# Vchitect/Latte

Measured on AMD Instinct MI355X. Metric: denoising steps/sec, higher is better.
Workload: dtype f16; 1 GPU; Latte-XL/2 FaceForensics (uncond) 16x256x256 -> latents 16x4x32x32, DDIM on the '250' respacing, random-init weights; per_gpu_batch=8, global_batch=8, parallelism=dp1 (independent samples)

## Files before the change

latte_amd/csrc/engine.cpp:

```cpp
#include <algorithm>
#include <cmath>
#include <cstdio>
#include <cstring>
#include <string>
#include <vector>

#include "event_profile.h"
#include "plan.h"
#include "weight_store.h"

namespace latte {

static thread_local std::string g_last_error;
static std::atomic<int> g_debug_choice[DBG_NUM_CHOICES];
int debug_choice(DebugChoice c) { return g_debug_choice[c].load(std::memory_order_relaxed); }
int set_debug_choice(const char* name, int value) {
  static const char* const names[DBG_NUM_CHOICES] = {"attn_variant", "xattn_flash", "tn_kernel", "tn_wn", "attn_bwd_tiles", "conv_kernel", "vae_split", "gated_rmw_shape"};
  static const int allowed[DBG_NUM_CHOICES][4] = {{1, 5, 12, 13}, {1, 0, 0, 0}, {4, 0, 0, 0}, {4, 0, 0, 0}, {1, 2, 0, 0}, {1, 2, 3, 4}, {0, 0, 0, 0}, {1, 2, 0, 0}};
  for (int i = 0; i < DBG_NUM_CHOICES; ++i) {
    if (name && std::string(name) == names[i]) {
      bool ok = value == 0;
      for (int k = 0; k < 4; ++k) ok = ok || (allowed[i][k] != 0 && value == allowed[i][k]);
      ok = ok || (i == DBG_VAE_SPLIT && (value >> 24) == 1);
      if (!ok) return -1;
// ... 199 lines not shown
  } else {
    if ((rc = launch_patch_embed(x, e->pe_wt, e->pe_b, e->pos, e->xres, B * F, e->Cin, e->H, c.patch_size, D, st))) return rc;
  }
  tm.mark(C_PATCH);
  int gsplit = cfg_dup ? e->guided_split : 0;
  if (dt != LATTE_DTYPE_F16) gsplit &= 3;
  if ((gsplit & 16) && !gemm_lo4_ok(M, e->Hm, D)) gsplit = (gsplit & ~16) | 8;
  if (gsplit & 16) gsplit &= ~10;
  if (gsplit & 4) gsplit &= ~1;
  if (gsplit & 8) gsplit &= ~2;
  if ((gsplit & 4) && !gemm_lo8_ok(M, D, D)) gsplit = (gsplit & ~4) | 1;
  if ((gsplit & 8) && !gemm_lo8_ok(M, e->Hm, D)) gsplit = (gsplit & ~8) | 2;
  if ((gsplit & 3) && (uint64_t)e->rows_pad * 2 * D * 2 >= (1ull << 32)) gsplit &= ~3;
  if (gsplit) gsplit = ensure_split_weights(e, gsplit, st);
  int gactive = gsplit & 26;

  for (int i = 0; i < c.depth; ++i) {
    const bool spatial = (i % 2) == 0;
    const BlockW& w = e->blocks[i];
    const float* mb = modp + (size_t)i * 6 * D;
    bool split_proj = false;
    const int fc2_variant = e->gemm_variant_of[3] ? e->gemm_variant_of[3] : e->gemm_variant;
    const bool te_in_fc2 = e->fc2_temp_embed && c.depth > 1 && gated_gemm_takes_te(e, M, D, e->Hm, fc2_variant);
    const float* te = (i == 1 && !te_in_fc2) ? e->temp : nullptr;
    if ((rc = launch_ln_modulate(e->xres, e->xres, e->xn, mb, mb + D, mstride, M, D, rps, te, T, F, dt, st))) return rc;
    tm.mark(C_LN);
    GemmArgs g{};
    g.M = M; g.rows_per_sample = rps; g.gate_stride = mstride; g.rmw_mode = e->gated_rmw_shape;
    const half_t* attn_out = e->xn;
    if (((e->fuse_qkv_attn >> (spatial ? 0 : 1)) & 1) && qkv_attention_fusable(D, c.num_heads, e->hd, F, T, spatial ? 0 : 1, M)) {
      QkvAttnArgs qa{};
      qa.xn = e->xn; qa.w = w.qkv_w; qa.bias = w.qkv_b; qa.out = e->qkv; qa.B = B; qa.F = F; qa.T = T; qa.D = D;
      qa.heads = c.num_heads; qa.hd = e->hd; qa.mode = spatial ? 0 : 1; qa.scale = 1.0f / std::sqrt((float)e->hd);
      qa.flags = ((e->fuse_qkv_attn >> 2) & 7) ^ 7;
      split_proj = gsplit & 5;
      qa.out_split = (gsplit & 4) ? 2 : (gsplit & 1);
      qa.out8 = e->lo8;
      gactive |= gsplit & 5;
      if ((rc = launch_qkv_attention(qa, dt, st))) return rc;
      tm.mark(spatial ? C_QKVATTN_S : C_QKVATTN_T);
      attn_out = e->qkv;
    } else {
      g.A = e->xn; g.W = w.qkv_w; g.bias = w.qkv_b; g.out = e->qkv; g.N = 3 * D; g.K = D;
      if ((rc = launch_gemm(g, EPI_BIAS_H16, dt, e->gemm_variant_of[0] ? e->gemm_variant_of[0] : e->gemm_variant, st))) return rc;
      tm.mark(C_QKV);
      AttnArgs a{};
      a.qkv = e->qkv; a.out = e->xn; a.heads = c.num_heads; a.hd = e->hd; a.D = D;
      a.sample_stride = rps; a.scale = 1.0f / std::sqrt((float)e->hd);
      if (spatial) { a.num_seq = B * F; a.L = T; a.U = F; a.seq_stride = T; a.row_stride = 1; }
      else         { a.num_seq = B * T; a.L = F; a.U = T; a.seq_stride = 1; a.row_stride = T; }
      if (gsplit & 4) {
        a.out8 = e->lo8;
        split_proj = true;
        gactive |= 4;
      }
      if ((rc = launch_attention(a, dt, st))) return rc;
      tm.mark(spatial ? C_ATTN_S : C_ATTN_T);
    }
    g.A = attn_out; g.W = w.proj_w; g.bias = w.proj_b; g.out = e->xres; g.gate = mb + 2 * D; g.N = D; g.K = D; g.tag = 0;
    if (split_proj && (gsplit & 4)) { g.A8 = e->lo8; g.W8 = w.proj_w8; }
    else if (split_proj) { g.W = w.proj_w2; g.K = 2 * D; }
    if ((rc = gated_gemm(e, g, dt, e->gemm_variant_of[1] ? e->gemm_variant_of[1] : e->gemm_variant, st))) return rc;
    g.A8 = nullptr; g.W8 = nullptr;
    tm.mark(C_PROJ);
    const int split_fc1 = (gsplit & 16) ? 3 : (gsplit & 8) ? 2 : (gsplit & 2) ? 1 : 0;
    if (split_fc1 == 3) rc = launch_ln_modulate_split4(e->xres, e->xn, e->lo4, e->lo4s, mb + 3 * D, mb + 4 * D, mstride, M, D, rps, dt, st);
    else rc = launch_ln_modulate(e->xres, e->xres, split_fc1 == 1 ? e->xn2 : e->xn, mb + 3 * D, mb + 4 * D, mstride, M, D, rps, nullptr, T, F, dt, st,
// ... 368 lines not shown
  const std::string k = name;
  if (k == "gemm_variant") {
    if (value < 0 || (value > 13 && value != 18 && value != 19)) return fail(LATTE_ERR_INVALID, "gemm_variant must be 0..13, 18 or 19");
    const int bn = value >= 7 && value <= 9 ? gemm_tile_n((int)value) / 4 : gemm_tile_n((int)value);
    if (value != 0 && ((3 * e->D) % bn || e->D % bn || e->Hm % bn))
      return fail(LATTE_ERR_INVALID, "gemm_variant: every N of the model must be a multiple of the tile width");
    e->gemm_variant = (int)value;
    return LATTE_OK;
  }
  for (int gi = 0; gi < 4; ++gi) {
    static const char* names[4] = {"gemm_variant_qkv", "gemm_variant_proj", "gemm_variant_fc1", "gemm_variant_fc2"};
    if (k == names[gi]) {
      if (value < 0 || (value > 13 && value != 18 && value != 19)) return fail(LATTE_ERR_INVALID, "gemm_variant_*: must be 0..13, 18 or 19");
      e->gemm_variant_of[gi] = (int)value;
      return LATTE_OK;
    }
  }
  if (k == "gated_split_k") {
    if (value < 0 || value > 4) return fail(LATTE_ERR_INVALID, "gated_split_k: 0 (rule), 1 (off) or 2..4 splits");
    e->gated_split_k = (int)value;
    return LATTE_OK;
  }
  if (k == "gated_rmw_shape") {
    if (value < 0 || value > 1) return fail(LATTE_ERR_INVALID, "gated_rmw_shape: 0 (fragment-wise) or 1 (line-wise residual accesses of the gated GEMMs)");
    e->gated_rmw_shape = (int)value;
    return LATTE_OK;
  }
  if (k == "fc2_temp_embed") {
    if (value < 0 || value > 1) return fail(LATTE_ERR_INVALID, "fc2_temp_embed: 0 (LayerNorm pass adds temp_embed) or 1 (the first block's fc2 epilogue does)");
    e->fc2_temp_embed = (int)value;
    return LATTE_OK;
  }
  if (k == "fuse_qkv_attn") {
    if (value < 0 || value > 31)
      return fail(LATTE_ERR_INVALID, "fuse_qkv_attn: bit 0 = spatial blocks, bit 1 = temporal blocks, bits 2-4 = schedule features off (0..31)");
    e->fuse_qkv_attn = (int)value;
    return LATTE_OK;
  }
  if (k == "guided_split") {
    if (value < 0 || value > 31)
      return fail(LATTE_ERR_INVALID, "guided_split: bit 0 / 1 = attention output / fc1 operand as f16 split pairs, bit 2 / 3 = the same with an fp8 remainder, bit 4 = fc1's operand with an fp4 remainder, in guided calls (0..31)");
    e->guided_split = (int)value;
    return LATTE_OK;
  }
  if (k == "seed") {
    e->seed = (uint64_t)value;
    e->rng_offset = 0;
    return LATTE_OK;
  }
  if (k == "train_timesteps") {
    if (value < 1 || value > (1 << 30)) return fail(LATTE_ERR_INVALID, "train_timesteps: the number of trained timesteps, >= 1");
    e->train_timesteps = (int)value;
    return LATTE_OK;
  }
  return fail(LATTE_ERR_INVALID, "set_option: unknown option '" + k + "'");
}

int latte_engine_get_option(const latte_engine_t* e, const char* name, int64_t* value) {
  if (!e || !name || !value) return fail(LATTE_ERR_INVALID, "get_option: null argument");
  const std::string k = name;
  if (k == "gemm_variant") *value = e->gemm_variant;
  else if (k == "gemm_variant_qkv") *value = e->gemm_variant_of[0];
  else if (k == "gemm_variant_proj") *value = e->gemm_variant_of[1];
  else if (k == "gemm_variant_fc1") *value = e->gemm_variant_of[2];
  else if (k == "gemm_variant_fc2") *value = e->gemm_variant_of[3];
  else if (k == "gated_split_k") *value = e->gated_split_k;
  else if (k == "gated_rmw_shape") *value = e->gated_rmw_shape;
  else if (k == "fc2_temp_embed") *value = e->fc2_temp_embed;
// ... 408 lines not shown
```

latte_amd/csrc/qkv_attn.hip:

```cpp
#include <type_traits>

#include "common.h"
#include "mfma_util.h"

namespace latte {
namespace {

constexpr int RPQ = 144, RPV = 160;
[[maybe_unused]] constexpr int Q_OFF = 0;
constexpr int K_OFF = 256 * RPQ, V_OFF = 2 * 256 * RPQ, IMG_END = V_OFF + 256 * RPV;
constexpr int A0_OFF = 0, A1_OFF = 61440, B1_OFF = 94208, B0_OFF = 122880, BIAS_OFF = B0_OFF + 224 * 128;
constexpr int FUSED_LDS = BIAS_OFF + 288 * 4;

__device__ __forceinline__ void rows_transpose4(unsigned int& x0, unsigned int& x1, unsigned int& x2, unsigned int& x3) {
  typedef __attribute__((ext_vector_type(2))) unsigned int u2;
  const u2 a = __builtin_amdgcn_permlane32_swap(x0, x2, false, false);
  const u2 b = __builtin_amdgcn_permlane32_swap(x1, x3, false, false);
  const u2 c = __builtin_amdgcn_permlane16_swap(a[0], b[0], false, false);
  const u2 d = __builtin_amdgcn_permlane16_swap(a[1], b[1], false, false);
  x0 = c[0]; x1 = c[1]; x2 = d[0]; x3 = d[1];
}

template <int HD, int DT, int MODE, int FLAGS, int SPLIT = 0>
__global__ void __launch_bounds__(512) qkv_attn_kernel(QkvAttnArgs a) {
  constexpr bool EARLY = (FLAGS & 1) != 0, PRIO = (FLAGS & 2) != 0;
  constexpr int NQ = 3 * HD;
  constexpr int NPAD = (NQ + 31) / 32 * 32;
  constexpr int FN = NPAD / 32;
  constexpr int B_MAIN = NPAD / 8 / 4;
  constexpr int GPM = HD / 8;
  constexpr int KS = (HD + 31) / 32, DF = (HD + 15) / 16, NCH = HD / 8;
  static_assert(NPAD <= 224 && NQ <= 288 && HD % 8 == 0 && A1_OFF >= 256 * 128 && B1_OFF - A1_OFF == 256 * 128 && B1_OFF + NPAD * 128 <= B0_OFF && IMG_END <= B0_OFF && K_OFF >= 256 * 128,
                "LDS plan");

  extern __shared__ __attribute__((aligned(16))) char smem[];
  const int lane = threadIdx.x & 63;
  const int wave = __builtin_amdgcn_readfirstlane(threadIdx.x >> 6);
  const int grp = wave >> 2, w4 = wave & 3, wm = w4 >> 1, wn = w4 & 1;
  const int D = a.D, T = a.T, F = a.F;
  const int out_ld = SPLIT == 1 ? 2 * D : D;
  const unsigned row_bytes = (unsigned)D * 2u;
  const int nk = D / 64;

  const int S = MODE == 0 ? a.B * F : a.B * (T >> 4);
  const bool xmap = (S & 7) == 0;
  const bool hmap = (a.flags & 4) != 0 && a.heads == 16 && xmap;
  const int xcd = blockIdx.x & 7;
  int it = xmap ? (int)(blockIdx.x >> 3) : (int)blockIdx.x;
  const int it_step = xmap ? (int)(gridDim.x >> 3) : (int)gridDim.x;
  const int it_end = xmap ? (S >> 3) * a.heads : S * a.heads;

  const __amdgpu_buffer_rsrc_t rsA =
      __builtin_amdgcn_make_buffer_rsrc((void*)a.xn, 0, (unsigned)((size_t)a.B * F * T) * row_bytes, 0x00020000);
  const __amdgpu_buffer_rsrc_t rsB = __builtin_amdgcn_make_buffer_rsrc((void*)a.w, 0, (unsigned)(3 * D) * row_bytes, 0x00020000);

  const int lrow = lane >> 3, cpos = lane & 7;
  const unsigned swz16 = (unsigned)((cpos ^ ((((w4 & 1) << 2) + (lrow >> 1)) & 7)) << 4);
  const unsigned voff_b = (unsigned)lrow * row_bytes + swz16;
// ... 97 lines not shown
    asm volatile("s_waitcnt lgkmcnt(0)" ::: "memory");
    __builtin_amdgcn_s_barrier();
    dma_a_half(cur, 1, 1);
    if (grp == 0) dma_b_all(cur, 1, 1);
    if (grp == 1) __builtin_amdgcn_s_barrier();
    for (int kt = 0; kt < nk; ++kt) {
      const char* sbuf_a = smem + ((kt & 1) ? A1_OFF : A0_OFF);
      const char* sbuf_b = smem + ((kt & 1) ? B1_OFF : B0_OFF);
      u32x4 bf[2][FN], af[2][4];
#pragma unroll
      for (int ks = 0; ks < 2; ++ks) {
#pragma unroll
        for (int j = 0; j < FN; ++j) bf[ks][j] = *(const u32x4*)(sbuf_b + ((b_off + j * 2048) ^ (ks << 6)));
#pragma unroll
        for (int i = 0; i < 4; ++i) af[ks][i] = *(const u32x4*)(sbuf_a + ((a_off + i * 2048) ^ (ks << 6)));
      }
      asm volatile("s_waitcnt lgkmcnt(0)" ::: "memory");
      __builtin_amdgcn_s_barrier();
      __builtin_amdgcn_s_setprio(1);
#pragma unroll
      for (int ks = 0; ks < 2; ++ks)
#pragma unroll
        for (int i = 0; i < 4; ++i)
#pragma unroll
          for (int j = 0; j < FN; ++j) acc[i][j] = mfma16<DT>(bf[ks][j], af[ks][i], acc[i][j]);
      __builtin_amdgcn_s_setprio(0);
      asm volatile("s_waitcnt vmcnt(0)" ::: "memory");
      __builtin_amdgcn_s_barrier();
      if (kt + 2 < nk) {
        dma_a_half(cur, kt + 2, kt & 1);
        if (grp == 0) dma_b_all(cur, kt + 2, kt & 1);
      }
    }
    if (grp == 0) __builtin_amdgcn_s_barrier();
    LATTE_PHASE(0)

    {
#pragma unroll
      for (int j = 0; j < FN; ++j) {
        const int n0 = wn * (NPAD / 2) + j * 16 + g * 4;
        if (n0 < NQ) {
          const int mat = n0 >= 2 * HD ? 2 : (n0 >= HD ? 1 : 0);
          const int d = n0 - mat * HD;
          const float4 b4 = *(const float4*)(smem + BIAS_OFF + n0 * 4);
          char* dst = smem + (mat == 2 ? V_OFF + (grp * 128 + wm * 64 + fr) * RPV : mat * K_OFF + (grp * 128 + wm * 64 + fr) * RPQ) + d * 2;
#pragma unroll
          for (int i = 0; i < 4; ++i) {
            const u32x2 pk = {pack2<DT>(acc[i][j][0] + b4.x, acc[i][j][1] + b4.y), pack2<DT>(acc[i][j][2] + b4.z, acc[i][j][3] + b4.w)};
            *(u32x2*)(dst + i * 16 * (mat == 2 ? RPV : RPQ)) = pk;
          }
        }
      }
    }
    __syncthreads();
    LATTE_PHASE(1)

    if (a.dbg_qkv != nullptr) {
      for (int idx = threadIdx.x; idx < 256 * 3 * NCH; idx += 512) {
        const int r = idx / (3 * NCH), rem = idx - r * (3 * NCH), mat = rem / NCH, ch = rem - mat * NCH;
        const int grow = MODE == 0 ? row_base + r : row_base + (r & 15) * T + (r >> 4);
        *(u32x4*)(a.dbg_qkv + (size_t)grow * (3 * D) + mat * D + head * HD + ch * 8) = *(const u32x4*)(smem + (mat == 2 ? V_OFF + r * RPV : mat * K_OFF + r * RPQ) + ch * 16);
      }
    }

    const char* q_img = smem;
    const char* k_img = smem + K_OFF;
    const char* v_img = smem + V_OFF;
    const float c = a.scale * 1.4426950408889634f;
    if constexpr (PRIO) {
      if (grp == 0) __builtin_amdgcn_s_setprio(2);
    }
    if constexpr (MODE == 0) {
      constexpr int NKT = 16;
      const int q0 = wave * 32;
      const char* kbase = k_img + fr * RPQ + g * 16;
      const char* vbase = v_img + (4 * g + (fr >> 2)) * RPV + (fr & 3) * 8;
      constexpr int NG = 2;
      {
        u32x4 qf[NG][KS];
#pragma unroll
        for (int gq = 0; gq < NG; ++gq)
#pragma unroll
          for (int ks = 0; ks < KS; ++ks) {
            const int ch = g + 4 * ks;
// ... 55 lines not shown
        for (int gq = 0; gq < NG; ++gq)
#pragma unroll
          for (int d = 0; d < DF; ++d) o[gq][d] = (f32x4){0.f, 0.f, 0.f, 0.f};
        u32x4 vfr[2][DF];
        auto load_v = [&](int ks2, u32x4 (&dst)[DF]) {
#pragma unroll
          for (int d = 0; d < DF; ++d) {
            const u32x2 lo = lds_tr16(vbase + (32 * ks2) * RPV + d * 32);
            const u32x2 hi = lds_tr16(vbase + (32 * ks2 + 16) * RPV + d * 32);
            dst[d] = (u32x4){lo[0], lo[1], hi[0], hi[1]};
          }
        };
        load_v(0, vfr[0]);
#pragma unroll
        for (int ks2 = 0; ks2 < NKT / 2; ++ks2) {
          if (ks2 + 1 < NKT / 2) load_v(ks2 + 1, vfr[(ks2 + 1) & 1]);
          u32x4 pb[NG];
#pragma unroll
          for (int gq = 0; gq < NG; ++gq)
            pb[gq] = (u32x4){pack2<DT>(st[gq][2 * ks2][0], st[gq][2 * ks2][1]), pack2<DT>(st[gq][2 * ks2][2], st[gq][2 * ks2][3]),
                             pack2<DT>(st[gq][2 * ks2 + 1][0], st[gq][2 * ks2 + 1][1]),
                             pack2<DT>(st[gq][2 * ks2 + 1][2], st[gq][2 * ks2 + 1][3])};
          __builtin_amdgcn_sched_barrier(0);
#pragma unroll
          for (int d = 0; d < DF; ++d)
#pragma unroll
            for (int gq = 0; gq < NG; ++gq) o[gq][d] = mfma16<DT>(vfr[ks2 & 1][d], pb[gq], o[gq][d]);
          __builtin_amdgcn_sched_barrier(0);
        }
#pragma unroll
        for (int gq = 0; gq < NG; ++gq) {
          half_t* orow = a.out + (size_t)(row_base + q0 + gq * 16 + fr) * out_ld + head * HD;
          unsigned int l8w[DF];
#pragma unroll
          for (int d = 0; d < DF; ++d) {
            const int dd = 16 * d + 4 * g;
            l8w[d] = 0u;
            if (dd < HD) {
              if constexpr (SPLIT == 1) {
                unsigned int h0_, l0_, h1_, l1_;
                split2<DT>(o[gq][d][0] * inv[gq], o[gq][d][1] * inv[gq], h0_, l0_);
                split2<DT>(o[gq][d][2] * inv[gq], o[gq][d][3] * inv[gq], h1_, l1_);
                const u32x2 hi = {h0_, h1_}, lo = {l0_, l1_};
                *(u32x2*)(orow + dd) = hi;
                *(u32x2*)(orow + D + dd) = lo;
              } else if constexpr (SPLIT == 2) {
                unsigned int h0_, h1_;
                l8w[d] = split8_f16(o[gq][d][0] * inv[gq], o[gq][d][1] * inv[gq], o[gq][d][2] * inv[gq], o[gq][d][3] * inv[gq], h0_, h1_);
                *(u32x2*)(orow + dd) = (u32x2){h0_, h1_};
              } else {
                const u32x2 pk = {pack2<DT>(o[gq][d][0] * inv[gq], o[gq][d][1] * inv[gq]),
                                  pack2<DT>(o[gq][d][2] * inv[gq], o[gq][d][3] * inv[gq])};
                *(u32x2*)(orow + dd) = pk;
              }
            }
          }
          if constexpr (SPLIT == 2) {
            unsigned char* o8 = a.out8 + (size_t)(row_base + q0 + gq * 16 + fr) * D + head * HD;
            rows_transpose4(l8w[0], l8w[1], l8w[2], l8w[3]);
            *(u32x4*)(o8 + 16 * g) = (u32x4){l8w[0], l8w[1], l8w[2], l8w[3]};
            if constexpr (DF > 4) { if (64 + 4 * g < HD) *(unsigned int*)(o8 + 64 + 4 * g) = l8w[4]; }
          }
        }
      }
    } else {
      f32x4 st2[2];
#pragma unroll
      for (int s2 = 0; s2 < 2; ++s2) {
        const int p = wave * 2 + s2;
        u32x4 qf[KS], kf[KS];
#pragma unroll
        for (int ks = 0; ks < KS; ++ks) {
          const int ch = g + 4 * ks;
          qf[ks] = *(const u32x4*)(q_img + (16 * p + fr) * RPQ + ch * 16);
          kf[ks] = *(const u32x4*)(k_img + (16 * p + fr) * RPQ + ch * 16);
          if (ch >= NCH) {
            qf[ks] = (u32x4){0u, 0u, 0u, 0u};
            kf[ks] = (u32x4){0u, 0u, 0u, 0u};
          }
        }
        st2[s2] = (f32x4){0.f, 0.f, 0.f, 0.f};
#pragma unroll
        for (int ks = 0; ks < KS; ++ks) st2[s2] = mfma16<DT>(kf[ks], qf[ks], st2[s2]);
      }
      early_fill();
#pragma unroll
      for (int s2 = 0; s2 < 2; ++s2) {
        const int p = wave * 2 + s2;
        f32x4 st = st2[s2];
        float mx = NEG_BIG;
#pragma unroll
        for (int r = 0; r < 4; ++r) mx = fmaxf(mx, st[r]);
        mx = fmaxf(mx, __shfl_xor(mx, 16, 64));
        mx = fmaxf(mx, __shfl_xor(mx, 32, 64));
        const float nm = -mx * c;
// ... 39 lines not shown
              *(u32x2*)(orow + dd) = pk;
            }
          }
        }
        if constexpr (SPLIT == 2) {
          unsigned char* o8 = a.out8 + (size_t)(row_base + fr * T + p) * D + head * HD;
          rows_transpose4(l8w[0], l8w[1], l8w[2], l8w[3]);
          *(u32x4*)(o8 + 16 * g) = (u32x4){l8w[0], l8w[1], l8w[2], l8w[3]};
          if constexpr (DF > 4) { if (64 + 4 * g < HD) *(unsigned int*)(o8 + 64 + 4 * g) = l8w[4]; }
        }
      }
    }
    if constexpr (PRIO) __builtin_amdgcn_s_setprio(0);
    asm volatile("s_waitcnt lgkmcnt(0)" ::: "memory");
    __builtin_amdgcn_s_barrier();
    LATTE_PHASE(2)
    tacc[3] += 1;
    if (!has_next) break;
    if (!filled_next) {
      fill_first(nxt);
      side = fetch_side(nxt);
    }
    cur = nxt;
    it = it_next;
  }
#undef LATTE_PHASE
  if (trace && lane == 0) {
    long long* o = a.dbg_trace + wave * 4;
#pragma unroll
    for (int i = 0; i < 4; ++i) o[i] = tacc[i];
  }
}

template <int HD, int DT, int MODE, int FLAGS, int SPLIT = 0>
int launch_one(const QkvAttnArgs& a, dim3 grid, hipStream_t st) {
  return launch_lds<qkv_attn_kernel<HD, DT, MODE, FLAGS, SPLIT>>(grid, dim3(512), FUSED_LDS, st, a);
}

template <int HD, int DT>
int launch_mode(const QkvAttnArgs& a, hipStream_t st) {
  const int S = a.mode == 0 ? a.B * a.F : a.B * (a.T >> 4);
  const int units = S * a.heads;
  const dim3 grid(units >= 256 ? 256 : (units + 7) / 8 * 8);
  if (a.out_split == 2) {
    if constexpr (DT == LATTE_DTYPE_F16) {
      if (!a.out8) return fail(LATTE_ERR_INVALID, "fused qkv + attention: out_split 2 needs out8");
      return a.mode == 0 ? launch_one<HD, DT, 0, 3, 2>(a, grid, st) : launch_one<HD, DT, 1, 1, 2>(a, grid, st);
    } else {
      return fail(LATTE_ERR_INVALID, "fused qkv + attention: the fp8-remainder output is f16 only");
    }
  }
  if (a.out_split)
    return a.mode == 0 ? launch_one<HD, DT, 0, 3, 1>(a, grid, st) : launch_one<HD, DT, 1, 1, 1>(a, grid, st);
  if (a.mode == 0) {
    switch (a.flags & 3) {
      case 0: return launch_one<HD, DT, 0, 0>(a, grid, st);
      case 1: return launch_one<HD, DT, 0, 1>(a, grid, st);
      case 2: return launch_one<HD, DT, 0, 2>(a, grid, st);
      default: return launch_one<HD, DT, 0, 3>(a, grid, st);
    }
  }
  return (a.flags & 1) ? launch_one<HD, DT, 1, 1>(a, grid, st) : launch_one<HD, DT, 1, 0>(a, grid, st);
}

}

bool qkv_attention_fusable(int D, int heads, int hd, int F, int T, int mode, int64_t rows) {
  if (heads * hd != D || (hd != 64 && hd != 72) || D % 64 != 0 || D < 128) return false;
  if ((uint64_t)rows * D * 2 >= (1ull << 32) || (uint64_t)3 * D * D * 2 >= (1ull << 32)) return false;
  if (mode == 0) return T == 256;
  return F == 16 && T % 16 == 0;
}

int launch_qkv_attention(const QkvAttnArgs& a, int dtype, hipStream_t st) {
  if (!qkv_attention_fusable(a.D, a.heads, a.hd, a.F, a.T, a.mode, (int64_t)a.B * a.F * a.T))
    return fail(LATTE_ERR_INVALID, "fused qkv + attention: shape not supported (need T == 256 spatial / F == 16 temporal, hd 64 | 72)");
  if (dtype == LATTE_DTYPE_BF16) return a.hd == 64 ? launch_mode<64, LATTE_DTYPE_BF16>(a, st) : launch_mode<72, LATTE_DTYPE_BF16>(a, st);
  if (dtype == LATTE_DTYPE_F16) return a.hd == 64 ? launch_mode<64, LATTE_DTYPE_F16>(a, st) : launch_mode<72, LATTE_DTYPE_F16>(a, st);
  return fail(LATTE_ERR_INVALID, "fused qkv + attention: unknown dtype");
}

}
```

latte_amd/csrc/t2v_engine.cpp:

```cpp
#include <algorithm>
#include <cmath>
#include <cstring>
#include <string>
#include <vector>

#include "../../include/latte_amd.h"
#include "plan.h"
#include "weight_store.h"

using namespace latte;

namespace {

enum T2VKind { TK_F32, TK_F32_TRANSPOSE, TK_H16 };

struct T2VBlock {
  half_t *qkv_w, *o_w, *q2_w, *kv2_w, *o2_w, *fc1_w, *fc2_w;
  float *qkv_b, *o_b, *q2_b, *kv2_b, *o2_b, *fc1_b, *fc2_b;
};

void sincos_1d(int dim, const std::vector<double>& pos, std::vector<double>& out ) {
  const int half = dim / 2, n = (int)pos.size();
  out.assign((size_t)n * dim, 0.0);
  for (int m = 0; m < n; ++m)
// ... 201 lines not shown
  LATTE_HIP(hipDeviceSynchronize());
  *out = e;
  return LATTE_OK;
}

void latte_t2v_destroy(latte_t2v_t* e) {
  delete e;
}

int latte_t2v_num_keys(const latte_t2v_t* e) { return e ? e->weights.size() : 0; }
const char* latte_t2v_key(const latte_t2v_t* e, int i) { return e ? e->weights.key(i) : nullptr; }

int latte_t2v_load_tensor(latte_t2v_t* e, const char* key, const float* data, int64_t numel, int on_device, void* stream) {
  if (!e || !key || !data) return fail(LATTE_ERR_INVALID, "t2v_load_tensor: null argument");
  hipStream_t st = (hipStream_t)stream;
  WeightSlot* slot = nullptr;
  const float* src = nullptr;
  int rc = e->weights.begin_load("t2v_load_tensor", key, data, numel, on_device, st, &slot, &src);
  if (rc || slot->optional) return rc;
  WeightSlot& s = *slot;
  switch (s.kind) {
    case TK_F32: LATTE_HIP(hipMemcpyAsync(s.dst, src, sizeof(float) * numel, hipMemcpyDeviceToDevice, st)); break;
    case TK_F32_TRANSPOSE: rc = launch_transpose_f32(src, (float*)s.dst, s.rows, s.cols, st); break;
    case TK_H16: rc = launch_convert_f32_to_h16(src, (half_t*)s.dst, numel, e->cfg.compute_dtype, st); break;
  }
  if (rc || (rc = e->weights.end_load(s, on_device, st))) return rc;
  e->txt_batch = 0;
  return LATTE_OK;
}

int latte_t2v_set_option(latte_t2v_t* e, const char* name, int64_t value) {
  if (!e || !name) return fail(LATTE_ERR_INVALID, "t2v_set_option: null argument");
  if (std::string(name) == "fuse_qkv_attn") {
    if (value < 0 || value > 31) return fail(LATTE_ERR_INVALID, "fuse_qkv_attn: bit 0 = spatial blocks, bit 1 = temporal blocks, bits 2-3 = schedule variant");
    e->fuse_qkv_attn = (int)value;
    return LATTE_OK;
  }
  return fail(LATTE_ERR_INVALID, std::string("t2v_set_option: unknown option '") + name + "'");
}

int latte_t2v_check_weights(latte_t2v_t* e) {
  if (!e) return fail(LATTE_ERR_INVALID, "t2v_check_weights: null engine");
  return e->weights.check_loaded();
}

static int t2v_text_context(latte_t2v* e, const float* enc, const float* mask, int B, int Lk, hipStream_t st) {
  const auto& c = e->cfg;
  const int D = e->D, dt = c.compute_dtype, MT = B * Lk;
  int rc;
  GemmArgs g{};
  g.rows_per_sample = MT; g.gate_stride = 0;
  if ((rc = launch_convert_f32_to_h16(enc, e->ctx_in, (int64_t)MT * e->Cc, dt, st))) return rc;
  g.M = MT; g.A = e->ctx_in; g.W = e->cap1_w; g.bias = e->cap1_b; g.out = e->ctx1; g.N = D; g.K = e->Cc;
  if ((rc = launch_gemm(g, EPI_BIAS_GELU_H16, dt, 0, st))) return rc;
  g.A = e->ctx1; g.W = e->cap2_w; g.bias = e->cap2_b; g.out = e->ctx; g.K = D;
  if ((rc = launch_gemm(g, EPI_BIAS_H16, dt, 0, st))) return rc;
  for (int l = 0; l < e->L; ++l) {
    const T2VBlock& w = e->blocks[2 * l];
    GemmArgs gk{};
    gk.M = MT; gk.rows_per_sample = MT; gk.A = e->ctx; gk.W = w.kv2_w; gk.bias = w.kv2_b;
    gk.out = e->kv_all + (size_t)l * e->trows_pad * 2 * D; gk.N = 2 * D; gk.K = D;
    if ((rc = launch_gemm(gk, EPI_BIAS_H16, dt, 0, st))) return rc;
  }
  e->txt_has_mask = mask != nullptr;
  if (mask && (rc = launch_mask_bias(mask, e->kbias, (size_t)MT, st))) return rc;
  e->txt_batch = B;
  e->txt_nk = Lk;
// ... 4 lines not shown
                    hipStream_t st) {
  const auto& c = e->cfg;
  const int D = e->D, T = e->T, F = e->F, dt = c.compute_dtype, Lk = e->txt_nk;
  const int M = B * F * T, rps = F * T;
  const int nt = t_shared ? 1 : B;
  const int mstride = t_shared ? 0 : (6 * e->nblk + 2) * D;
  const float* kbias = e->txt_has_mask ? e->kbias : nullptr;
  int rc;
  if ((rc = launch_small_linear(IN_TFREQ, nullptr, t, e->t1_w, e->t1_b, nullptr, nullptr, e->temb0, nt, D, 256, D, st))) return rc;
  if ((rc = launch_small_linear(IN_SILU, e->temb0, nullptr, e->t2_w, e->t2_b, nullptr, nullptr, e->temb, nt, D, D, D, st))) return rc;
  if ((rc = launch_small_linear(IN_SILU, e->temb, nullptr, e->ada_w, e->ada_b, nullptr, nullptr, e->t6, nt, 6 * D, D, 6 * D, st))) return rc;
  if ((rc = launch_adaln_single(e->tables, e->head_table, e->t6, e->temb, e->mod, nt, e->nblk, D, st))) return rc;
  const int xb = dup ? B / 2 : B;
  if ((rc = launch_permute_cf(x, e->xin, xb, c.in_channels, F, e->H * e->H, 1, st))) return rc;
  if ((rc = launch_patch_embed(e->xin, e->pe_wt, e->pe_b, e->pos, e->xres, xb * F, c.in_channels, e->H, c.patch_size, D, st))) return rc;
  if (dup && (rc = launch_patch_embed(e->xin, e->pe_wt, e->pe_b, e->pos, e->xres + (size_t)xb * rps * D, xb * F, c.in_channels,
                                      e->H, c.patch_size, D, st))) return rc;

  GemmArgs g{};
  for (int i = 0; i < e->nblk; ++i) {
    const bool spatial = (i % 2) == 0;
    if (!spatial && !enable_temporal) continue;
    const T2VBlock& w = e->blocks[i];
    const float* mb = e->mod + (size_t)i * 6 * D;
    const float* te = (i == 1 && F > 1) ? e->temp : nullptr;
    if ((rc = launch_ln_modulate(e->xres, e->xres, e->xn, mb, mb + D, mstride, M, D, rps, te, T, F, dt, st))) return rc;
    g = GemmArgs{};
    g.M = M; g.rows_per_sample = rps; g.gate_stride = mstride;
    const half_t* attn_out = e->xn;
    const float attn_scale = 1.0f / std::sqrt((float)e->hd);
    if (((e->fuse_qkv_attn >> (spatial ? 0 : 1)) & 1) && qkv_attention_fusable(D, e->heads, e->hd, F, T, spatial ? 0 : 1, M)) {
      QkvAttnArgs qa{};
      qa.xn = e->xn; qa.w = w.qkv_w; qa.bias = w.qkv_b; qa.out = e->qkv; qa.B = B; qa.F = F; qa.T = T; qa.D = D;
      qa.heads = e->heads; qa.hd = e->hd; qa.mode = spatial ? 0 : 1; qa.scale = attn_scale; qa.flags = ((e->fuse_qkv_attn >> 2) & 7) ^ 7;
      if ((rc = launch_qkv_attention(qa, dt, st))) return rc;
      attn_out = e->qkv;
    } else {
      g.A = e->xn; g.W = w.qkv_w; g.bias = w.qkv_b; g.out = e->qkv; g.N = 3 * D; g.K = D;
      if ((rc = launch_gemm(g, EPI_BIAS_H16, dt, 0, st))) return rc;
      AttnArgs a{};
      a.qkv = e->qkv; a.out = e->xn; a.heads = e->heads; a.hd = e->hd; a.D = D;
      a.sample_stride = rps; a.scale = attn_scale;
      if (spatial) { a.num_seq = B * F; a.L = T; a.U = F; a.seq_stride = T; a.row_stride = 1; }
      else         { a.num_seq = B * T; a.L = F; a.U = T; a.seq_stride = 1; a.row_stride = T; }
      if ((rc = launch_attention(a, dt, st))) return rc;
    }
    g.A = attn_out; g.W = w.o_w; g.bias = w.o_b; g.out = e->xres; g.gate = mb + 2 * D; g.N = D; g.K = D; g.tag = 0;
    if ((rc = launch_gemm(g, EPI_GATE_RES_F32, dt, 0, st))) return rc;
    if (spatial) {
      if ((rc = launch_convert_f32_to_h16(e->xres, e->xn, (int64_t)M * D, dt, st))) return rc;
      g.A = e->xn; g.W = w.q2_w; g.bias = w.q2_b; g.out = e->qkv; g.gate = nullptr; g.N = D; g.K = D;
      if ((rc = launch_gemm(g, EPI_BIAS_H16, dt, 0, st))) return rc;
      AttnArgs x2{};
      x2.qkv = e->qkv; x2.q_ld = D; x2.kv = e->kv_all + (size_t)(i / 2) * e->trows_pad * 2 * D; x2.kbias = kbias; x2.Lk = Lk;
      x2.out = e->xn;
      x2.heads = e->heads; x2.hd = e->hd; x2.D = D; x2.sample_stride = rps; x2.scale = attn_scale;
      x2.num_seq = B * F; x2.L = T; x2.U = F; x2.seq_stride = T; x2.row_stride = 1;
      if ((rc = launch_cross_attention(x2, dt, st))) return rc;
      g.A = e->xn; g.W = w.o2_w; g.bias = w.o2_b; g.out = e->xres; g.gate = e->ones; g.gate_stride = 0; g.N = D; g.K = D;
      if ((rc = launch_gemm(g, EPI_GATE_RES_F32, dt, 0, st))) return rc;
      g.gate_stride = mstride;
    }
    if ((rc = launch_ln_modulate(e->xres, e->xres, e->xn, mb + 3 * D, mb + 4 * D, mstride, M, D, rps, nullptr, T, F, dt, st))) return rc;
    g.A = e->xn; g.W = w.fc1_w; g.bias = w.fc1_b; g.out = e->hbuf; g.gate = nullptr; g.N = e->Hm; g.K = D;
    if ((rc = launch_gemm(g, EPI_BIAS_GELU_H16, dt, 0, st))) return rc;
    g.A = e->hbuf; g.W = w.fc2_w; g.bias = w.fc2_b; g.out = e->xres; g.gate = mb + 5 * D; g.N = D; g.K = e->Hm; g.tag = 1;
    if ((rc = launch_gemm(g, EPI_GATE_RES_F32, dt, 0, st))) return rc;
// ... 108 lines not shown
```

Measured before the change: 266.6 sample-steps/s.

## Restructure fused QKV-attention epilogue writes and temporal attention phase with cross-lane permutes

The fused QKV+attention kernel now preloads bias vectors into registers before the image-write phase. It also rewrites the attention-output store so fragments are gathered across lanes with permlane swaps into full 16-byte row writes. A new temporal-mode path processes two sequences per wave: V transposes are issued early, and softmax max/sum reductions use permlane16/32 swaps instead of LDS or shuffle traffic. The old paths stay reachable through new option bits 5-6, which adds template instantiations and compile time.

Result: no change. 267.6 sample-steps/s (median of 6 runs) (+0.4%).

```diff
diff --git a/latte_amd/csrc/engine.cpp b/latte_amd/csrc/engine.cpp
--- a/latte_amd/csrc/engine.cpp
+++ b/latte_amd/csrc/engine.cpp
@@ -255,7 +255,7 @@
       QkvAttnArgs qa{};
       qa.xn = e->xn; qa.w = w.qkv_w; qa.bias = w.qkv_b; qa.out = e->qkv; qa.B = B; qa.F = F; qa.T = T; qa.D = D;
       qa.heads = c.num_heads; qa.hd = e->hd; qa.mode = spatial ? 0 : 1; qa.scale = 1.0f / std::sqrt((float)e->hd);
-      qa.flags = ((e->fuse_qkv_attn >> 2) & 7) ^ 7;
+      qa.flags = (((e->fuse_qkv_attn >> 2) & 7) ^ 7) | (((e->fuse_qkv_attn >> 5) & 3) << 3);
       split_proj = gsplit & 5;
       qa.out_split = (gsplit & 4) ? 2 : (gsplit & 1);
       qa.out8 = e->lo8;
@@ -690,8 +690,8 @@
     return LATTE_OK;
   }
   if (k == "fuse_qkv_attn") {
-    if (value < 0 || value > 31)
-      return fail(LATTE_ERR_INVALID, "fuse_qkv_attn: bit 0 = spatial blocks, bit 1 = temporal blocks, bits 2-4 = schedule features off (0..31)");
+    if (value < 0 || value > 127)
+      return fail(LATTE_ERR_INVALID, "fuse_qkv_attn: bit 0 = spatial blocks, bit 1 = temporal blocks, bits 2-4 = schedule features off, bits 5-6 = image-write / temporal attention phase as before (0..127)");
     e->fuse_qkv_attn = (int)value;
     return LATTE_OK;
   }
diff --git a/latte_amd/csrc/qkv_attn.hip b/latte_amd/csrc/qkv_attn.hip
--- a/latte_amd/csrc/qkv_attn.hip
+++ b/latte_amd/csrc/qkv_attn.hip
@@ -21,9 +21,44 @@
   x0 = c[0]; x1 = c[1]; x2 = d[0]; x3 = d[1];
 }
 
-template <int HD, int DT, int MODE, int FLAGS, int SPLIT = 0>
+__device__ __forceinline__ u32x4 rows_gather2(u32x2 a, u32x2 b) {
+  typedef __attribute__((ext_vector_type(2))) unsigned int u2;
+  const u2 l = __builtin_amdgcn_permlane32_swap(a[0], b[0], false, false);
+  const u2 h = __builtin_amdgcn_permlane32_swap(a[1], b[1], false, false);
+  const u2 l2 = __builtin_amdgcn_permlane16_swap(l[0], l[1], false, false);
+  const u2 h2 = __builtin_amdgcn_permlane16_swap(h[0], h[1], false, false);
+  return (u32x4){l2[0], h2[0], l2[1], h2[1]};
+}
+
+__device__ __forceinline__ void xor_pair16(float v, float& r0, float& r1) {
+  typedef __attribute__((ext_vector_type(2))) unsigned int u2;
+  const unsigned int b = __builtin_bit_cast(unsigned int, v);
+  const u2 r = __builtin_amdgcn_permlane16_swap(b, b, false, false);
+  const unsigned int w0 = r[0], w1 = r[1];
+  r0 = __builtin_bit_cast(float, w0); r1 = __builtin_bit_cast(float, w1);
+}
+__device__ __forceinline__ void xor_pair32(float v, float& r0, float& r1) {
+  typedef __attribute__((ext_vector_type(2))) unsigned int u2;
+  const unsigned int b = __builtin_bit_cast(unsigned int, v);
+  const u2 r = __builtin_amdgcn_permlane32_swap(b, b, false, false);
+  const unsigned int w0 = r[0], w1 = r[1];
+  r0 = __builtin_bit_cast(float, w0); r1 = __builtin_bit_cast(float, w1);
+}
+__device__ __forceinline__ float max_rows4(float v) {
+  float r0, r1;
+  xor_pair16(v, r0, r1); v = fmaxf(r0, r1);
+  xor_pair32(v, r0, r1); return fmaxf(r0, r1);
+}
+__device__ __forceinline__ float sum_rows4(float v) {
+  float r0, r1;
+  xor_pair16(v, r0, r1); v = r0 + r1;
+  xor_pair32(v, r0, r1); return r0 + r1;
+}
+
+template <int HD, int DT, int MODE, int FLAGS, int SPLIT = 0, int OLD = 0>
 __global__ void __launch_bounds__(512) qkv_attn_kernel(QkvAttnArgs a) {
   constexpr bool EARLY = (FLAGS & 1) != 0, PRIO = (FLAGS & 2) != 0;
+  constexpr bool OLD_E = (OLD & 1) != 0, OLD_A = (OLD & 2) != 0;
   constexpr int NQ = 3 * HD;
   constexpr int NPAD = (NQ + 31) / 32 * 32;
   constexpr int FN = NPAD / 32;
@@ -187,6 +222,11 @@
         if (grp == 0) dma_b_all(cur, kt + 2, kt & 1);
       }
     }
+    [[maybe_unused]] float4 bq[FN];
+    if constexpr (!OLD_E) {
+#pragma unroll
+      for (int j = 0; j < FN; ++j) bq[j] = *(const float4*)(smem + BIAS_OFF + (wn * (NPAD / 2) + j * 16 + g * 4) * 4);
+    }
     if (grp == 0) __builtin_amdgcn_s_barrier();
     LATTE_PHASE(0)
 
@@ -197,7 +237,9 @@
         if (n0 < NQ) {
           const int mat = n0 >= 2 * HD ? 2 : (n0 >= HD ? 1 : 0);
           const int d = n0 - mat * HD;
-          const float4 b4 = *(const float4*)(smem + BIAS_OFF + n0 * 4);
+          float4 b4;
+          if constexpr (OLD_E) b4 = *(const float4*)(smem + BIAS_OFF + n0 * 4);
+          else b4 = bq[j];
           char* dst = smem + (mat == 2 ? V_OFF + (grp * 128 + wm * 64 + fr) * RPV : mat * K_OFF + (grp * 128 + wm * 64 + fr) * RPQ) + d * 2;
 #pragma unroll
           for (int i = 0; i < 4; ++i) {
@@ -205,6 +247,7 @@
             *(u32x2*)(dst + i * 16 * (mat == 2 ? RPV : RPQ)) = pk;
           }
         }
+        if constexpr (!OLD_E) __builtin_amdgcn_sched_barrier(0);
       }
     }
     __syncthreads();
@@ -326,8 +369,34 @@
         for (int gq = 0; gq < NG; ++gq) {
           half_t* orow = a.out + (size_t)(row_base + q0 + gq * 16 + fr) * out_ld + head * HD;
           unsigned int l8w[DF];
-#pragma unroll
-          for (int d = 0; d < DF; ++d) {
+          if constexpr (!OLD_A) {
+            u32x2 hw[4];
+            [[maybe_unused]] u32x2 lw[4];
+#pragma unroll
+            for (int d = 0; d < 4; ++d) {
+              l8w[d] = 0u;
+              if constexpr (SPLIT == 1) {
+                unsigned int h0_, l0_, h1_, l1_;
+                split2<DT>(o[gq][d][0] * inv[gq], o[gq][d][1] * inv[gq], h0_, l0_);
+                split2<DT>(o[gq][d][2] * inv[gq], o[gq][d][3] * inv[gq], h1_, l1_);
+                hw[d] = (u32x2){h0_, h1_};
+                lw[d] = (u32x2){l0_, l1_};
+              } else if constexpr (SPLIT == 2) {
+                unsigned int h0_, h1_;
+                l8w[d] = split8_f16(o[gq][d][0] * inv[gq], o[gq][d][1] * inv[gq], o[gq][d][2] * inv[gq], o[gq][d][3] * inv[gq], h0_, h1_);
+                hw[d] = (u32x2){h0_, h1_};
+              } else {
+                hw[d] = (u32x2){pack2<DT>(o[gq][d][0] * inv[gq], o[gq][d][1] * inv[gq]), pack2<DT>(o[gq][d][2] * inv[gq], o[gq][d][3] * inv[gq])};
+              }
+            }
+#pragma unroll
+            for (int pr = 0; pr < 2; ++pr) {
+              *(u32x4*)(orow + 32 * pr + 8 * g) = rows_gather2(hw[2 * pr], hw[2 * pr + 1]);
+              if constexpr (SPLIT == 1) *(u32x4*)(orow + D + 32 * pr + 8 * g) = rows_gather2(lw[2 * pr], lw[2 * pr + 1]);
+            }
+          }
+#pragma unroll
+          for (int d = OLD_A ? 0 : 4; d < DF; ++d) {
             const int dd = 16 * d + 4 * g;
             l8w[d] = 0u;
             if (dd < HD) {
@@ -355,6 +424,133 @@
             *(u32x4*)(o8 + 16 * g) = (u32x4){l8w[0], l8w[1], l8w[2], l8w[3]};
             if constexpr (DF > 4) { if (64 + 4 * g < HD) *(unsigned int*)(o8 + 64 + 4 * g) = l8w[4]; }
           }
+        }
+      }
+    } else if constexpr (!OLD_A) {
+      u32x2 vf[2][5];
+#pragma unroll
+      for (int s2 = 0; s2 < 2; ++s2) {
+        const char* vp = v_img + (16 * (wave * 2 + s2) + 4 * g + (fr >> 2)) * RPV + (fr & 3) * 8;
+        vf[s2][0] = lds_tr16_asm<0>(vp); vf[s2][1] = lds_tr16_asm<32>(vp); vf[s2][2] = lds_tr16_asm<64>(vp);
+        vf[s2][3] = lds_tr16_asm<96>(vp); vf[s2][4] = lds_tr16_asm<128>(vp);
+      }
+      __builtin_amdgcn_sched_barrier(0);
+      u32x4 qf[2][KS], kf[2][KS];
+#pragma unroll
+      for (int s2 = 0; s2 < 2; ++s2) {
+        const int p = wave * 2 + s2;
+#pragma unroll
+        for (int ks = 0; ks < KS; ++ks) {
+          const int ch = g + 4 * ks;
+          qf[s2][ks] = *(const u32x4*)(q_img + (16 * p + fr) * RPQ + ch * 16);
+          kf[s2][ks] = *(const u32x4*)(k_img + (16 * p + fr) * RPQ + ch * 16);
+          if (ch >= NCH) {
+            qf[s2][ks] = (u32x4){0u, 0u, 0u, 0u};
+            kf[s2][ks] = (u32x4){0u, 0u, 0u, 0u};
+          }
+        }
+      }
+      f32x4 st[2] = {(f32x4){0.f, 0.f, 0.f, 0.f}, (f32x4){0.f, 0.f, 0.f, 0.f}};
+#pragma unroll
+      for (int ks = 0; ks < KS; ++ks)
+#pragma unroll
+        for (int s2 = 0; s2 < 2; ++s2) st[s2] = mfma16<DT>(kf[s2][ks], qf[s2][ks], st[s2]);
+      asm volatile("s_waitcnt lgkmcnt(0)"
+                   : "+v"(vf[0][0]), "+v"(vf[0][1]), "+v"(vf[0][2]), "+v"(vf[0][3]), "+v"(vf[0][4]), "+v"(vf[1][0]), "+v"(vf[1][1]),
+                     "+v"(vf[1][2]), "+v"(vf[1][3]), "+v"(vf[1][4])
+                   :
+                   : "memory");
+      early_fill();
+      float mx[2], ls[2], inv[2];
+      u32x2 pb[2];
+#pragma unroll
+      for (int s2 = 0; s2 < 2; ++s2) {
+        mx[s2] = NEG_BIG;
+#pragma unroll
+        for (int r = 0; r < 4; ++r) mx[s2] = fmaxf(mx[s2], st[s2][r]);
+      }
+#pragma unroll
+      for (int s2 = 0; s2 < 2; ++s2) mx[s2] = max_rows4(mx[s2]);
+#pragma unroll
+      for (int s2 = 0; s2 < 2; ++s2) {
+        const float nm = -mx[s2] * c;
+        ls[s2] = 0.f;
+#pragma unroll
+        for (int r = 0; r < 4; ++r) {
+          st[s2][r] = __builtin_amdgcn_exp2f(__builtin_fmaf(st[s2][r], c, nm));
+          ls[s2] += st[s2][r];
+        }
+      }
+#pragma unroll
+      for (int s2 = 0; s2 < 2; ++s2) {
+        ls[s2] = sum_rows4(ls[s2]);
+        pb[s2] = (u32x2){pack2<DT>(st[s2][0], st[s2][1]), pack2<DT>(st[s2][2], st[s2][3])};
+        inv[s2] = 1.0f / ls[s2];
+      }
+      f32x4 o[2][DF];
+#pragma unroll
+      for (int d = 0; d < DF; ++d)
+#pragma unroll
+        for (int s2 = 0; s2 < 2; ++s2) o[s2][d] = mfma16_k16<DT>(vf[s2][d], pb[s2], (f32x4){0.f, 0.f, 0.f, 0.f});
+#pragma unroll
+      for (int s2 = 0; s2 < 2; ++s2) {
+        const int p = wave * 2 + s2;
+        half_t* orow = a.out + (size_t)(row_base + fr * T + p) * out_ld + head * HD;
+        unsigned int l8w[DF];
+        u32x2 hw[4];
+        [[maybe_unused]] u32x2 lw[4];
+#pragma unroll
+        for (int d = 0; d < 4; ++d) {
+          const f32x4 oacc = o[s2][d];
+          const float inv_ = inv[s2];
+          l8w[d] = 0u;
+          if constexpr (SPLIT == 1) {
+            unsigned int h0_, l0_, h1_, l1_;
+            split2<DT>(oacc[0] * inv_, oacc[1] * inv_, h0_, l0_);
+            split2<DT>(oacc[2] * inv_, oacc[3] * inv_, h1_, l1_);
+            hw[d] = (u32x2){h0_, h1_};
+            lw[d] = (u32x2){l0_, l1_};
+          } else if constexpr (SPLIT == 2) {
+            unsigned int h0_, h1_;
+            l8w[d] = split8_f16(oacc[0] * inv_, oacc[1] * inv_, oacc[2] * inv_, oacc[3] * inv_, h0_, h1_);
+            hw[d] = (u32x2){h0_, h1_};
+          } else {
+            hw[d] = (u32x2){pack2<DT>(oacc[0] * inv_, oacc[1] * inv_), pack2<DT>(oacc[2] * inv_, oacc[3] * inv_)};
+          }
+        }
+#pragma unroll
+        for (int pr = 0; pr < 2; ++pr) {
+          *(u32x4*)(orow + 32 * pr + 8 * g) = rows_gather2(hw[2 * pr], hw[2 * pr + 1]);
+          if constexpr (SPLIT == 1) *(u32x4*)(orow + D + 32 * pr + 8 * g) = rows_gather2(lw[2 * pr], lw[2 * pr + 1]);
+        }
+        if constexpr (DF > 4) {
+          const f32x4 oacc = o[s2][4];
+          const float inv_ = inv[s2];
+          const int dd = 64 + 4 * g;
+          l8w[4] = 0u;
+          if (dd < HD) {
+            if constexpr (SPLIT == 1) {
+              unsigned int h0_, l0_, h1_, l1_;
+              split2<DT>(oacc[0] * inv_, oacc[1] * inv_, h0_, l0_);
+              split2<DT>(oacc[2] * inv_, oacc[3] * inv_, h1_, l1_);
+              const u32x2 hi = {h0_, h1_}, lo = {l0_, l1_};
+              *(u32x2*)(orow + dd) = hi;
+              *(u32x2*)(orow + D + dd) = lo;
+            } else if constexpr (SPLIT == 2) {
+              unsigned int h0_, h1_;
+              l8w[4] = split8_f16(oacc[0] * inv_, oacc[1] * inv_, oacc[2] * inv_, oacc[3] * inv_, h0_, h1_);
+              *(u32x2*)(orow + dd) = (u32x2){h0_, h1_};
+            } else {
+              const u32x2 pk = {pack2<DT>(oacc[0] * inv_, oacc[1] * inv_), pack2<DT>(oacc[2] * inv_, oacc[3] * inv_)};
+              *(u32x2*)(orow + dd) = pk;
+            }
+          }
+        }
+        if constexpr (SPLIT == 2) {
+          unsigned char* o8 = a.out8 + (size_t)(row_base + fr * T + p) * D + head * HD;
+          rows_transpose4(l8w[0], l8w[1], l8w[2], l8w[3]);
+          *(u32x4*)(o8 + 16 * g) = (u32x4){l8w[0], l8w[1], l8w[2], l8w[3]};
+          if constexpr (DF > 4) { if (64 + 4 * g < HD) *(unsigned int*)(o8 + 64 + 4 * g) = l8w[4]; }
         }
       }
     } else {
@@ -460,9 +656,17 @@
   }
 }
 
-template <int HD, int DT, int MODE, int FLAGS, int SPLIT = 0>
+template <int HD, int DT, int MODE, int FLAGS, int SPLIT = 0, int OLD = 0>
 int launch_one(const QkvAttnArgs& a, dim3 grid, hipStream_t st) {
-  return launch_lds<qkv_attn_kernel<HD, DT, MODE, FLAGS, SPLIT>>(grid, dim3(512), FUSED_LDS, st, a);
+  return launch_lds<qkv_attn_kernel<HD, DT, MODE, FLAGS, SPLIT, OLD>>(grid, dim3(512), FUSED_LDS, st, a);
+}
+
+template <int HD, int DT, int MODE, int FLAGS>
+int launch_plain(const QkvAttnArgs& a, dim3 grid, hipStream_t st) {
+  const int old = (a.flags >> 3) & 3;
+  if (old == 3) return launch_one<HD, DT, MODE, FLAGS, 0, 3>(a, grid, st);
+  if (old == 2) return launch_one<HD, DT, MODE, FLAGS, 0, 2>(a, grid, st);
+  return old == 1 ? launch_one<HD, DT, MODE, FLAGS, 0, 1>(a, grid, st) : launch_one<HD, DT, MODE, FLAGS, 0, 0>(a, grid, st);
 }
 
 template <int HD, int DT>
@@ -482,13 +686,13 @@
     return a.mode == 0 ? launch_one<HD, DT, 0, 3, 1>(a, grid, st) : launch_one<HD, DT, 1, 1, 1>(a, grid, st);
   if (a.mode == 0) {
     switch (a.flags & 3) {
-      case 0: return launch_one<HD, DT, 0, 0>(a, grid, st);
-      case 1: return launch_one<HD, DT, 0, 1>(a, grid, st);
-      case 2: return launch_one<HD, DT, 0, 2>(a, grid, st);
-      default: return launch_one<HD, DT, 0, 3>(a, grid, st);
+      case 0: return launch_plain<HD, DT, 0, 0>(a, grid, st);
+      case 1: return launch_plain<HD, DT, 0, 1>(a, grid, st);
+      case 2: return launch_plain<HD, DT, 0, 2>(a, grid, st);
+      default: return launch_plain<HD, DT, 0, 3>(a, grid, st);
     }
   }
-  return (a.flags & 1) ? launch_one<HD, DT, 1, 1>(a, grid, st) : launch_one<HD, DT, 1, 0>(a, grid, st);
+  return (a.flags & 1) ? launch_plain<HD, DT, 1, 1>(a, grid, st) : launch_plain<HD, DT, 1, 0>(a, grid, st);
 }
 
 }
diff --git a/latte_amd/csrc/t2v_engine.cpp b/latte_amd/csrc/t2v_engine.cpp
--- a/latte_amd/csrc/t2v_engine.cpp
+++ b/latte_amd/csrc/t2v_engine.cpp
@@ -257,7 +257,7 @@
 int latte_t2v_set_option(latte_t2v_t* e, const char* name, int64_t value) {
   if (!e || !name) return fail(LATTE_ERR_INVALID, "t2v_set_option: null argument");
   if (std::string(name) == "fuse_qkv_attn") {
-    if (value < 0 || value > 31) return fail(LATTE_ERR_INVALID, "fuse_qkv_attn: bit 0 = spatial blocks, bit 1 = temporal blocks, bits 2-3 = schedule variant");
+    if (value < 0 || value > 127) return fail(LATTE_ERR_INVALID, "fuse_qkv_attn: bit 0 = spatial blocks, bit 1 = temporal blocks, bits 2-4 = schedule features off, bits 5-6 = image-write / temporal attention phase as before (0..127)");
     e->fuse_qkv_attn = (int)value;
     return LATTE_OK;
   }
@@ -328,7 +328,8 @@
     if (((e->fuse_qkv_attn >> (spatial ? 0 : 1)) & 1) && qkv_attention_fusable(D, e->heads, e->hd, F, T, spatial ? 0 : 1, M)) {
       QkvAttnArgs qa{};
       qa.xn = e->xn; qa.w = w.qkv_w; qa.bias = w.qkv_b; qa.out = e->qkv; qa.B = B; qa.F = F; qa.T = T; qa.D = D;
-      qa.heads = e->heads; qa.hd = e->hd; qa.mode = spatial ? 0 : 1; qa.scale = attn_scale; qa.flags = ((e->fuse_qkv_attn >> 2) & 7) ^ 7;
+      qa.heads = e->heads; qa.hd = e->hd; qa.mode = spatial ? 0 : 1; qa.scale = attn_scale;
+      qa.flags = (((e->fuse_qkv_attn >> 2) & 7) ^ 7) | (((e->fuse_qkv_attn >> 5) & 3) << 3);
       if ((rc = launch_qkv_attention(qa, dt, st))) return rc;
       attn_out = e->qkv;
     } else {
```
